# germannp/yalla

Hardware: AMD Instinct MI355X
Metric: cell-updates/sec at 1M cells (Grid_solver) (higher is better)
Workload: dtype f32

## Files before the change

include/solvers.cuh:

```cuda
#pragma once

#include <hip/hip_runtime.h>
#include <hip/hip_ext.h>

#include <assert.h>
#include <math.h>
#include <stdio.h>
#include <stdlib.h>
#include <string.h>

#include <functional>
#include <mutex>
#include <type_traits>
#include <utility>
#include <vector>

#include "cudebug.cuh"
#include "dtypes.cuh"
#include "fold256.cuh"
#include "yalla_hip.h"

#ifndef YALLA_NO_THRUST
#include <thrust/execution_policy.h>
#include <thrust/fill.h>
// ... 214 lines not shown

template<typename Pt>
__device__ __forceinline__ Pt store_rhs(
    Pt* __restrict__ d_dX, int i, bool has_gen, Pt F, float3 sum_v, float sum_friction)
{
    Pt dX;
    if (has_gen) {
        dX = d_dX[i];
        dX += F;
    } else {
        dX = F;
    }
    if (sum_friction > 0) {
        dX.x += sum_v.x / sum_friction;
        dX.y += sum_v.y / sum_friction;
        dX.z += sum_v.z / sum_friction;
    }
    d_dX[i] = dX;
    return dX;
}

template<typename Pt, Pairwise_interaction<Pt> pw_int, Pairwise_friction<Pt> pw_friction>
__device__ __forceinline__ void tile_pair(const Pt Xi, const Pt& Xj, const float3& vj, const int i, const int j, Pt& F,
    float3& sum_v, float& sum_friction)
{
    Pt r = Xi - Xj;
    float dist = dist3(r.x, r.y, r.z);
    F += pw_int(Xi, r, dist, i, j);
    float friction = pw_friction(Xi, r, dist, i, j);
    sum_friction += friction;
    if (friction != 0) {
        float3 v = vj;
        sum_v.x += friction * v.x;
        sum_v.y += friction * v.y;
        sum_v.z += friction * v.z;
    }
}

template<typename Pt, Pairwise_interaction<Pt> pw_int, Pairwise_friction<Pt> pw_friction>
__device__ __forceinline__ void tile_force_rows(const int n, const int block, const int id_base,
    const Pt* __restrict__ d_X, const float3* __restrict__ d_old_v, Pt* __restrict__ d_dX, const bool has_gen)
{
    __shared__ Pt sh_X[TILE_POINTS];
    __shared__ float3 sh_v[TILE_POINTS];

    const int local = block * TILE_BLOCK + threadIdx.x;
    const int i = id_base + local;
    Pt Xi = ya::zero<Pt>();
    if (local < n) Xi = d_X[local];
    Pt F = ya::zero<Pt>();
    float3 sum_v{0.f, 0.f, 0.f};
    float sum_friction = 0;
    for (int tile_start = 0; tile_start < n; tile_start += TILE_POINTS) {
        const int n_tile = min(TILE_POINTS, n - tile_start);
        __syncthreads();
        for (int k = threadIdx.x; k < n_tile; k += TILE_BLOCK) {
            sh_X[k] = d_X[tile_start + k];
            sh_v[k] = d_old_v[tile_start + k];
        }
        __syncthreads();
        if (local < n) {
#ifndef YA_TILE_UNROLL
#define YA_TILE_UNROLL 4
#endif
#pragma unroll YA_TILE_UNROLL
            for (int k = 0; k < n_tile; k++) {
                const int j = id_base + tile_start + k;
                tile_pair<Pt, pw_int, pw_friction>(Xi, sh_X[k], sh_v[k], i, j, F, sum_v, sum_friction);
            }
        }
    }
    if (local < n) store_rhs(d_dX, local, has_gen, F, sum_v, sum_friction);
}
template<typename Pt, Pairwise_interaction<Pt> pw_int, Pairwise_friction<Pt> pw_friction>
__global__ __launch_bounds__(TILE_BLOCK) void tile_force(const int n,
    const Pt* __restrict__ d_X, const float3* __restrict__ d_old_v, Pt* __restrict__ d_dX,
    const bool has_gen)
{
    tile_force_rows<Pt, pw_int, pw_friction>(n, blockIdx.x, 0, d_X, d_old_v, d_dX, has_gen);
}

template<typename Pt, Pairwise_interaction<Pt> pw_int, Pairwise_friction<Pt> pw_friction, int COOP_LANES>
__device__ __forceinline__ void tile_force_coop_rows(const int n, const int block, const int id_base,
    const Pt* __restrict__ d_X, const float3* __restrict__ d_old_v, Pt* __restrict__ d_dX, const bool has_gen)
{
    constexpr int COOP_CELLS = 256 / COOP_LANES;
    constexpr int NF = N_floats<Pt>::value;
    constexpr int NC = NF + 4;
    constexpr int TILE = (57344 / (COOP_CELLS * NC * 4)) / 64 * 64 > 512 ? 512 : (57344 / (COOP_CELLS * NC * 4)) / 64 * 64;
    static_assert(TILE >= 64, "point type too large for tile_force_coop");
    constexpr int THREADS = COOP_CELLS * COOP_LANES;
    constexpr int LOADS = (TILE + THREADS - 1) / THREADS;
    constexpr int SLOTS = (NC + COOP_LANES - 1) / COOP_LANES;
    __shared__ __attribute__((aligned(16))) float sh_part[COOP_CELLS][NC][TILE];
    __shared__ Pt sh_X[TILE];
    __shared__ float3 sh_v[TILE];
    __shared__ float sh_sum[COOP_CELLS][NC];

    const int cell = threadIdx.x / COOP_LANES, lane = threadIdx.x % COOP_LANES;
    const int local = block * COOP_CELLS + cell;
    const int i = id_base + local;
    const bool active = local < n;
    Pt Xi = ya::zero<Pt>();
    if (active) Xi = d_X[local];
    float acc[SLOTS];
#pragma unroll
    for (int a = 0; a < SLOTS; a++) acc[a] = 0.f;

    Pt x_next[LOADS];
    float3 v_next[LOADS];
#pragma unroll
    for (int k = 0; k < LOADS; k++) {
        const int j = threadIdx.x + k * THREADS;
        x_next[k] = ya::zero<Pt>();
        v_next[k] = float3{0.f, 0.f, 0.f};
        if (j < TILE && j < n) {
            x_next[k] = d_X[j];
            v_next[k] = d_old_v[j];
        }
    }
    for (int tile_start = 0; tile_start < n; tile_start += TILE) {
        const int n_tile = min(TILE, n - tile_start);
#pragma unroll
        for (int k = 0; k < LOADS; k++) {
            const int t = threadIdx.x + k * THREADS;
            if (t < TILE) {
                sh_X[t] = x_next[k];
                sh_v[t] = v_next[k];
                const int j_next = tile_start + TILE + t;
                if (j_next < n) {
                    x_next[k] = d_X[j_next];
                    v_next[k] = d_old_v[j_next];
                }
            }
        }
        __syncthreads();
        if (active) {
#pragma unroll 4
            for (int jj = lane; jj < n_tile; jj += COOP_LANES) {
                const int j = id_base + tile_start + jj;
                Pt r = Xi - sh_X[jj];
                float dist = dist3(r.x, r.y, r.z);
                const Pt f = pw_int(Xi, r, dist, i, j);
                const float friction = pw_friction(Xi, r, dist, i, j);
#pragma unroll
                for (int c = 0; c < NF; c++) sh_part[cell][c][jj] = field(f, c);
                sh_part[cell][NF][jj] = friction;
                const float3 v = sh_v[jj];
                sh_part[cell][NF + 1][jj] = friction != 0 ? friction * v.x : 0.f;
                sh_part[cell][NF + 2][jj] = friction != 0 ? friction * v.y : 0.f;
                sh_part[cell][NF + 3][jj] = friction != 0 ? friction * v.z : 0.f;
            }
        }
        __syncthreads();
#pragma unroll
        for (int a = 0; a < SLOTS; a++) {
            const int c = lane + COOP_LANES * a;
            if (c < NC && active) {
                float sum = acc[a];
                const float4* terms = reinterpret_cast<const float4*>(&sh_part[cell][c][0]);
                int jj = 0;
                for (; jj + 16 <= n_tile; jj += 16) {
                    float4 p[4];
#pragma unroll
                    for (int u = 0; u < 4; u++) p[u] = terms[jj / 4 + u];
#pragma unroll
                    for (int u = 0; u < 4; u++) {
                        sum += p[u].x;
                        sum += p[u].y;
                        sum += p[u].z;
                        sum += p[u].w;
                    }
                }
                for (; jj < n_tile; jj++) sum += sh_part[cell][c][jj];
                acc[a] = sum;
            }
        }
        __syncthreads();
    }
#pragma unroll
    for (int a = 0; a < SLOTS; a++) {
        const int c = lane + COOP_LANES * a;
        if (c < NC) sh_sum[cell][c] = acc[a];
    }
    __syncthreads();
    if (active && lane == 0) {
        Pt F;
#pragma unroll
        for (int c = 0; c < NF; c++) field(F, c) = sh_sum[cell][c];
        store_rhs(d_dX, local, has_gen, F,
            float3{sh_sum[cell][NF + 1], sh_sum[cell][NF + 2], sh_sum[cell][NF + 3]}, sh_sum[cell][NF]);
    }
}
template<typename Pt, Pairwise_interaction<Pt> pw_int, Pairwise_friction<Pt> pw_friction, int COOP_LANES>
__global__ __launch_bounds__(256) void tile_force_coop(const int n,
    const Pt* __restrict__ d_X, const float3* __restrict__ d_old_v, Pt* __restrict__ d_dX,
    const bool has_gen)
{
    tile_force_coop_rows<Pt, pw_int, pw_friction, COOP_LANES>(n, blockIdx.x, 0, d_X, d_old_v, d_dX, has_gen);
}

__device__ __forceinline__ int stencil_row_offset(int row, int gs)
{
    const int dy = row % 3, dz = row / 3;
    const int oy = dy == 0 ? 0 : (dy == 1 ? -gs : gs);
    const int oz = dz == 0 ? 0 : (dz == 1 ? -gs * gs : gs * gs);
    return oy + oz;
}


template<typename Pt>
__device__ __forceinline__ float4 staged_words(const Entry<Pt>* e)
{
    if constexpr (sizeof(Entry<Pt>) % 16 == 0)
        return *reinterpret_cast<const float4*>(e);
    else
        return float4{e->X.x, e->X.y, e->X.z, 0.f};
}
__device__ __forceinline__ void keep_wide(const float4& w) { asm volatile("" ::"v"(w.w)); }

template<typename Pt>
__device__ __forceinline__ float dist2_to(const Pt& a, const float4 b)
{
    const float dx = a.x - b.x;
    const float dy = a.y - b.y;
    const float dz = a.z - b.z;
    return fmaf(dz, dz, fmaf(dy, dy, dx * dx));
}

template<typename Pt>
__device__ __forceinline__ float dist2(const Pt& a, const Pt& b)
{
    const float dx = a.x - b.x;
    const float dy = a.y - b.y;
    const float dz = a.z - b.z;
    return fmaf(dz, dz, fmaf(dy, dy, dx * dx));
}

inline float cutoff_squared(float cube_size)
{
    float t = cube_size * cube_size;
    while (t > 0 && sqrtf(t) >= cube_size) t = nextafterf(t, 0.f);
    while (sqrtf(t) < cube_size) t = nextafterf(t, INFINITY);
    return t;
}

#ifndef YA_CALL_INLINED
#define YA_CALL_INLINED [[clang::always_inline]]
#endif

#define YA_ROW_BOUNDS(plane_)                                                          \
    _Pragma("unroll") for (int r = 0; r < 3; r++)                                      \
    {                                                                                  \
        const int off = stencil_row_offset(3 * (plane_) + r, gs);                      \
         \
         \
        next_lo[r] = offs[min(max(c_lo + off - 1, 0), n_cubes)];                       \
        next_hi[r] = offs[min(max(c_hi + off + 2, 0), n_cubes)];                       \
        next_begin[r] = offs[min(max(c + off - 1, 0), n_cubes)];                       \
        next_end[r] = offs[min(max(c + off + 2, 0), n_cubes)];                         \
    }

}
#ifdef YA_EXPERIMENTAL_FORCE_VARIANTS
#include "force_variants.cuh"
#endif
namespace ya {

template<typename Pt, Pairwise_friction<Pt> pw_friction>
__device__ __forceinline__ void pair_friction(const Pt& Xi, const Pt& r, const float dist, const int i,
    const int j, const float4& v, float3& sum_v, float& sum_friction)
{
    if constexpr (pw_friction == &friction_w_neighbour<Pt>) {
        const bool nb = (i != j) & (dist < 1.f);
        const float f = nb ? 1.f : 0.f;
        sum_friction += f;
        sum_v.x = fmaf(f, v.x, sum_v.x);
        sum_v.y = fmaf(f, v.y, sum_v.y);
        sum_v.z = fmaf(f, v.z, sum_v.z);
    } else {
        const float friction = pw_friction(Xi, r, dist, i, j);
        sum_friction += friction;
        if (friction != 0) {
            sum_v.x += friction * v.x;
            sum_v.y += friction * v.y;
            sum_v.z += friction * v.z;
        }
    }
}

#ifndef YA_BITS_PROBE_BEGIN
#define YA_BITS_PROBE_BEGIN
#define YA_BITS_PROBE_END(tile_)
#endif
namespace bits {
#ifndef YA_BITS_BLOCK
#define YA_BITS_BLOCK 64
#endif
#ifndef YA_MASK_WORDS
#define YA_MASK_WORDS 4
#endif
#ifndef YA_BITS_POPS
#define YA_BITS_POPS 2
#endif
#ifndef YA_BITS_POPS_WIDE
#define YA_BITS_POPS_WIDE 2
#endif
#ifndef YA_BITS_MIN_WAVES_WIDE
#define YA_BITS_MIN_WAVES_WIDE 1
#endif
template<typename Pt>
struct Min_waves {
    static constexpr int value = sizeof(Pt) <= 16 ? 1 : YA_BITS_MIN_WAVES_WIDE;
};
template<typename Pt>
struct Pops {
    static constexpr int value = sizeof(Pt) <= 16 ? YA_BITS_POPS : YA_BITS_POPS_WIDE;
};
constexpr int BLOCK = YA_BITS_BLOCK;
constexpr int WORDS = YA_MASK_WORDS;
constexpr int PASS_BITS = 32 * WORDS;
static_assert(BLOCK % 32 == 0, "phase 2 steps its word pointer by BLOCK / 32 elements per bit position");
using Lds_word = __attribute__((address_space(3))) unsigned;

template<typename Pt>
struct Stage {
#ifndef YA_BITS_STAGE_CELLS
#define YA_BITS_STAGE_CELLS (3 * YA_BITS_BLOCK + 160)
#endif
    static constexpr int value = sizeof(Entry<Pt>) <= 24 ? YA_BITS_STAGE_CELLS
                                 : (sizeof(Entry<Pt>) <= 32 ? 256 : YA_BITS_STAGE_CELLS / 2);
};

__device__ __forceinline__ void shift_in(unsigned& m, const float d2, const float cut2)
{
    asm("v_cmp_gt_f32 vcc, %2, %1\n\tv_addc_co_u32 %0, vcc, %0, %0, vcc"
        : "+v"(m)
        : "v"(d2), "s"(cut2)
        : "vcc");
}

__host__ __device__ constexpr bool offsets_fit_32_bits(const long long n)
{
    return n >= 0 && 16ll * n < (1ll << 32);
}

template<typename Pt, Pairwise_interaction<Pt> pw_int, Pairwise_friction<Pt> pw_friction, bool STAGE_V, bool GLOBAL_IDS,
    bool OFF32>
__device__ __forceinline__ void pass(const Entry<Pt>* __restrict__ sh_e, const float4* __restrict__ sh_v,
    Lds_word* const words,
    const int b0, const int e0, const int b1, const int e1, const int b2, const int e2,
    const int shift0, const int shift1, const int shift2, const float4* __restrict__ sorted_v,
    const Pt& Xi, const int i, const float cut2, Pt& F, float3& sum_v, float& sum_friction,
    const int* __restrict__ global_id, const int id_base = 0)
{
    constexpr int POPS = Pops<Pt>::value;
    unsigned m = 0;
    int p = 0;
    Lds_word* mp = words;
#define YA_BITS_GROUP(end_, masked_)                                                   \
    {                                                                                  \
        float4 w[4];                                                                   \
        float d2[4];                                                                   \
        _Pragma("unroll") for (int u = 0; u < 4; u++) w[u] = staged_words(&sh_e[t + u]); \
        _Pragma("unroll") for (int u = 0; u < 4; u++)                                  \
        {                                                                              \
            d2[u] = dist2_to(Xi, w[u]);                                                \
            keep_wide(w[u]);                                                           \
            if (masked_) d2[u] = t + u < (end_) ? d2[u] : INFINITY;                    \
        }                                                                              \
        _Pragma("unroll") for (int u = 0; u < 4; u++) shift_in(m, d2[u], cut2);        \
        p += 4;                                                                        \
        *mp = m;   \
        const bool full = (p & 31) == 0;                                               \
        mp += full ? BLOCK : 0;                                                        \
        m = full ? 0u : m;                                                             \
    }
#define YA_BITS_SEGMENT(begin_, end_)                                                  \
    {                                                                                  \
        int t = (begin_);                                                              \
        for (; t + 4 <= (end_); t += 4) YA_BITS_GROUP(end_, false)                     \
        if (t < (end_)) YA_BITS_GROUP(end_, true)                                      \
    }
    const int d0 = b0;
    YA_BITS_SEGMENT(b0, e0)
    const int p1 = p, d1 = b1 - p1;
    YA_BITS_SEGMENT(b1, e1)
    const int p2 = p, d2_ = b2 - p2;
    YA_BITS_SEGMENT(b2, e2)
#undef YA_BITS_SEGMENT
#undef YA_BITS_GROUP
    if (p & 31) *mp = m << (32 - (p & 31));

    constexpr unsigned ENTRY = sizeof(Entry<Pt>);
    constexpr bool ONE_OFFSET = ENTRY == sizeof(float4);
    const unsigned lds0 = ENTRY * (unsigned)d0, lds1 = ENTRY * (unsigned)d1, lds2 = ENTRY * (unsigned)d2_;
    const unsigned gat0 = 16u * (unsigned)(d0 + shift0), gat1 = 16u * (unsigned)(d1 + shift1),
                   gat2 = 16u * (unsigned)(d2_ + shift2);
    Lds_word* const rp_end = words + ((p + 31) >> 5) * BLOCK;
    unsigned cur = p > 0 ? words[0] : 0u;
    Lds_word* rp = words + BLOCK;
    unsigned nxt = *rp;
    int wbase = 0;
#define YA_BITS_LOAD(q_, other_, v_)                                                   \
    {                                                                                  \
        const bool in2 = (q_) >= p2, in1 = (q_) >= p1;                                 \
        if constexpr (OFF32 && ONE_OFFSET) {                                           \
            const unsigned at = ENTRY * (unsigned)(q_) + (in2 ? lds2 : (in1 ? lds1 : lds0)); \
            other_ = *(const Entry<Pt>*)((const char*)sh_e + at);                      \
            if (STAGE_V) v_ = *(const float4*)((const char*)sh_v + at);                \
        } else {                                                                       \
            const int t = (q_) + (in2 ? d2_ : (in1 ? d1 : d0));                        \
            other_ = sh_e[t];                                                          \
            if (STAGE_V) v_ = sh_v[t];                                                 \
            if (!STAGE_V && !OFF32) v_ = sorted_v[(unsigned)(t + (in2 ? shift2 : (in1 ? shift1 : shift0)))]; \
        }                                                                              \
        if constexpr (OFF32 && !STAGE_V) {                                             \
            const unsigned at = 16u * (unsigned)(q_) + (in2 ? gat2 : (in1 ? gat1 : gat0)); \
            v_ = *(const float4*)((const char*)sorted_v + (size_t)at);                 \
        }                                                                              \
    }
#define YA_BITS_PAIR(other_, v_)                                                       \
    {                                                                                  \
        Pt r = Xi - other_.X;                                                          \
        float dist = dist3(r.x, r.y, r.z);                                             \
        const int j = (GLOBAL_IDS ? global_id[other_.id] : other_.id) + id_base;       \
        YA_CALL_INLINED F += pw_int(Xi, r, dist, i, j);                                \
        pair_friction<Pt, pw_friction>(Xi, r, dist, i, j, v_, sum_v, sum_friction);    \
    }
#ifdef YA_BITS_MEASUREMENT_PROBES
#include "bits_probe.inc"
#endif
    while (cur != 0 || rp < rp_end) {
        const int step = cur == 0 ? 32 : 0;
        cur = cur == 0 ? nxt : cur;
        wbase += step;
        rp += step * (BLOCK / 32);
        nxt = *rp;
        if (cur != 0) {
            int pos[POPS];
            bool have[POPS];
            Entry<Pt> other[POPS];
            float4 v[POPS];
#pragma unroll
            for (int u = 0; u < POPS; u++) {
                have[u] = cur != 0;
                pos[u] = have[u] ? __builtin_clz(cur) : pos[u > 0 ? u - 1 : 0];
                cur = have[u] ? cur & (0x7fffffffu >> pos[u]) : cur;
                YA_BITS_LOAD(wbase + pos[u], other[u], v[u])
            }
            YA_BITS_PAIR(other[0], v[0])
#pragma unroll
            for (int u = 1; u < POPS; u++)
                if (have[u]) YA_BITS_PAIR(other[u], v[u])
        }
    }
#undef YA_BITS_LOAD
#undef YA_BITS_PAIR
}
}

template<typename Pt, Pairwise_interaction<Pt> pw_int, Pairwise_friction<Pt> pw_friction, bool STAGE_V, bool GLOBAL_IDS,
    bool OFF32>
__device__ __forceinline__ void grid_force_bits_tile(const int n, const int tile, const int id_base, const int half,
    const int slot, const Entry<Pt>* sorted, const float4* sorted_v,
    const int* cube_id, const int* offs, const int gs, const int n_cubes, const float cut2,
    Pt* d_dX, const bool has_gen, const int n_active, Pt* d_dX_sorted,
    const int* global_id, float* tail_exchange, int* tail_tickets, const bool by_plane);

template<typename Pt, Pairwise_interaction<Pt> pw_int, Pairwise_friction<Pt> pw_friction, bool STAGE_V = false,
    bool GLOBAL_IDS = false, bool OFF32 = true>
__global__ __launch_bounds__(bits::BLOCK, bits::Min_waves<Pt>::value) void grid_force_bits(const int n,
    const Entry<Pt>* __restrict__ sorted, const float4* __restrict__ sorted_v,
    const int* __restrict__ cube_id, const int* __restrict__ offs, const int gs,
    const int n_cubes, const float cut2, Pt* __restrict__ d_dX, const bool has_gen,
    const int n_active, Pt* __restrict__ d_dX_sorted, const int* __restrict__ global_id, const int n_tiles,
    const int tail, float* tail_exchange, int* tail_tickets, const bool by_plane,
    const int part = 0, const int part_cube_lo = 0, const int part_cube_hi = 0, const int own_cube_lo = 0,
    const int own_cube_hi = 0x7fffffff)
{
    constexpr int FB = bits::BLOCK;

    int tile, mine, t_first = 0, t_lo = 0, t_hi = 0;
    if (part == 0) {
        mine = n_tiles;
    } else {
        const int tiles = n_tiles;
        t_first = min(offs[min(max(own_cube_lo, 0), n_cubes)] / FB, tiles);
        const int t_end = max(min((offs[min(own_cube_hi, n_cubes)] + FB - 1) / FB, tiles), t_first);
        t_lo = max(min((offs[min(part_cube_lo, n_cubes)] + FB - 1) / FB, t_end), t_first);
        t_hi = max(min(offs[min(part_cube_hi, n_cubes)] / FB, t_end), t_lo);
        mine = part == 1 ? (t_lo - t_first) + (t_end - t_hi) : t_hi - t_lo;
    }
    const int whole = tail < 0 ? 0 : (tail > 0 && (part == 0 || mine >= 4 * tail) ? max(mine - tail, 0) & ~7 : mine);
    int half = -1, compact = blockIdx.x;
    if (compact >= whole) {
        const int b = compact - whole;
        half = (b >> 3) & 1;
        compact = whole + (b >> 4) * 8 + (b & 7);
    }
    if (compact >= mine) return;
    if (part == 0) {
        tile = xcd_contiguous_tile(compact, mine);
    } else {
        const int t = xcd_contiguous_tile<16>(compact, mine);
        if (part == 1)
            tile = t < t_lo - t_first ? t_first + t : t_hi + (t - (t_lo - t_first));
        else
            tile = t_lo + t;
    }
    grid_force_bits_tile<Pt, pw_int, pw_friction, STAGE_V, GLOBAL_IDS, OFF32>(n, tile, 0, half, compact - whole, sorted,
        sorted_v, cube_id, offs, gs, n_cubes, cut2, d_dX, has_gen, n_active, d_dX_sorted, global_id, tail_exchange,
        tail_tickets, by_plane);
}

template<typename Pt, Pairwise_interaction<Pt> pw_int, Pairwise_friction<Pt> pw_friction, bool STAGE_V, bool GLOBAL_IDS,
    bool OFF32>
__device__ __forceinline__ void grid_force_bits_tile(const int n, const int tile, const int id_base, const int half,
    const int slot, const Entry<Pt>* sorted, const float4* sorted_v,
    const int* cube_id, const int* offs, const int gs, const int n_cubes, const float cut2,
    Pt* d_dX, const bool has_gen, const int n_active, Pt* d_dX_sorted,
    const int* global_id, float* tail_exchange, int* tail_tickets, const bool by_plane)
{
    constexpr int FB = bits::BLOCK;
    constexpr int CAP = bits::Stage<Pt>::value;
    constexpr int NF = N_floats<Pt>::value;
    constexpr int NC = NF + 4;
    __shared__ __attribute__((aligned(16))) Entry<Pt> sh_e[CAP + 8];
    __shared__ unsigned sh_m[(bits::WORDS + 1) * FB];
    __shared__ float4 sh_v[STAGE_V ? CAP + 8 : 1];
    bits::Lds_word* const words = (bits::Lds_word*)sh_m + threadIdx.x;
    const int s0 = tile * FB;
    const int s = s0 + threadIdx.x;
    bool active = s < n;
    const int c_lo = cube_id[s0];
    const int c_hi = cube_id[min(s0 + FB, n) - 1];
    YA_BITS_PROBE_BEGIN

    Pt Xi = ya::zero<Pt>();
    int i = 0, c = c_lo;
    if (active) {
        const Entry<Pt> self = sorted[s];
        Xi = self.X;
        i = self.id;
        c = cube_id[s];
        active = i < n_active;
    }
    if (!__syncthreads_or(active)) return;
    const int gi = (GLOBAL_IDS && active ? global_id[i] : i) + id_base;
    Pt F = ya::zero<Pt>();
    float3 sum_v{0.f, 0.f, 0.f};
    float sum_friction = 0;

    constexpr bool OWN_IN_LDS = sizeof(Pt) > 16;
    __shared__ float sh_own[OWN_IN_LDS ? NC * FB : 1];
    float own[OWN_IN_LDS ? 1 : NC];
#pragma unroll
    for (int k = 0; k < (OWN_IN_LDS ? 1 : NC); k++) own[k] = 0.f;

    int next_lo[3], next_hi[3], next_begin[3], next_end[3];
    const int plane_first = half == 1 ? 1 : 0, plane_end = half == 0 ? 1 : 3;
#pragma unroll 1
    for (int plane = plane_first; plane < plane_end; plane++) {
        if (by_plane && half < 0 && plane == 1) {
            float save[NC];
#pragma unroll
            for (int k = 0; k < NF; k++) save[k] = field(F, k);
            save[NF] = sum_v.x, save[NF + 1] = sum_v.y, save[NF + 2] = sum_v.z, save[NF + 3] = sum_friction;
#pragma unroll
            for (int k = 0; k < NC; k++) {
                if (OWN_IN_LDS)
                    sh_own[k * FB + threadIdx.x] = save[k];
                else
                    own[OWN_IN_LDS ? 0 : k] = save[k];
            }
            F = ya::zero<Pt>(), sum_v = float3{0.f, 0.f, 0.f}, sum_friction = 0;
        }
        int wg_begin[3], v0[4], k_begin[3], k_end[3];
        v0[0] = 0;
        YA_ROW_BOUNDS(plane)
#pragma unroll
        for (int r = 0; r < 3; r++) {
            wg_begin[r] = next_lo[r];
            v0[r + 1] = v0[r] + next_hi[r] - wg_begin[r];
            k_begin[r] = next_begin[r];
            k_end[r] = active ? next_end[r] : k_begin[r];
        }
        const int total = v0[3];

        for (int chunk = 0; chunk < total; chunk += CAP) {
            const int chunk_n = min(CAP, total - chunk);
            __syncthreads();
            for (int t = threadIdx.x; t < chunk_n; t += FB) {
                const int v = chunk + t;
                const int shift = v >= v0[2] ? wg_begin[2] - v0[2]
                                             : (v >= v0[1] ? wg_begin[1] - v0[1] : wg_begin[0]);
                sh_e[t] = sorted[v + shift];
                if (STAGE_V) sh_v[t] = sorted_v[v + shift];
            }
            __syncthreads();
            int sb[3], se[3], shift[3];
#pragma unroll
            for (int r = 0; r < 3; r++) {
                sb[r] = max(k_begin[r] - wg_begin[r] + v0[r], chunk) - chunk;
                se[r] = min(k_end[r] - wg_begin[r] + v0[r], chunk + chunk_n) - chunk;
                shift[r] = wg_begin[r] - v0[r] + chunk;
            }
            const int bits_needed = (max(se[0] - sb[0], 0) + 3 & ~3) + (max(se[1] - sb[1], 0) + 3 & ~3) +
                                    (max(se[2] - sb[2], 0) + 3 & ~3);
            if (!__any(bits_needed > bits::PASS_BITS)) {
                bits::pass<Pt, pw_int, pw_friction, STAGE_V, GLOBAL_IDS, OFF32>(sh_e, sh_v, words, sb[0], se[0], sb[1], se[1], sb[2],
                    se[2], shift[0], shift[1], shift[2], sorted_v, Xi, gi, cut2, F, sum_v, sum_friction,
                    global_id, id_base);
            } else {
#pragma unroll 1
                for (int r = 0; r < 3; r++) {
                    const int rb = r == 0 ? sb[0] : (r == 1 ? sb[1] : sb[2]);
                    const int re = r == 0 ? se[0] : (r == 1 ? se[1] : se[2]);
                    const int rs = r == 0 ? shift[0] : (r == 1 ? shift[1] : shift[2]);
#pragma unroll 1
                    for (int b = rb; __any(b < re); b += bits::PASS_BITS)
                        bits::pass<Pt, pw_int, pw_friction, STAGE_V, GLOBAL_IDS, OFF32>(sh_e, sh_v, words, b, min(re, b + bits::PASS_BITS),
                            0, 0, 0, 0, rs, 0, 0, sorted_v, Xi, gi, cut2, F, sum_v, sum_friction, global_id, id_base);
                }
            }
        }
    }
    float sums[NC];
#pragma unroll
    for (int k = 0; k < NF; k++) sums[k] = field(F, k);
    sums[NF] = sum_v.x, sums[NF + 1] = sum_v.y, sums[NF + 2] = sum_v.z, sums[NF + 3] = sum_friction;
    if (half < 0) {
        if (by_plane) {
#pragma unroll
            for (int k = 0; k < NC; k++)
                sums[k] = (OWN_IN_LDS ? sh_own[k * FB + threadIdx.x] : own[OWN_IN_LDS ? 0 : k]) + sums[k];
        }
    } else {
        __shared__ int sh_second;
        float* const mine_out = tail_exchange + ((size_t)slot * 2 + half) * NC * FB + threadIdx.x;
#pragma unroll
        for (int k = 0; k < NC; k++)
            __hip_atomic_store(mine_out + k * FB, sums[k], __ATOMIC_RELAXED, __HIP_MEMORY_SCOPE_AGENT);
        asm volatile("s_waitcnt vmcnt(0)" ::: "memory");
        __syncthreads();
        if (threadIdx.x == 0)
            sh_second = __hip_atomic_fetch_add(&tail_tickets[slot], 1, __ATOMIC_RELAXED, __HIP_MEMORY_SCOPE_AGENT);
        __syncthreads();
        if (sh_second == 0) {
            YA_BITS_PROBE_END(tile)
            return;
        }
        if (threadIdx.x == 0) __hip_atomic_store(&tail_tickets[slot], 0, __ATOMIC_RELAXED, __HIP_MEMORY_SCOPE_AGENT);
        const float* const theirs = tail_exchange + ((size_t)slot * 2 + (1 - half)) * NC * FB + threadIdx.x;
#pragma unroll
        for (int k = 0; k < NC; k++)
            sums[k] = sums[k] + __hip_atomic_load(theirs + k * FB, __ATOMIC_RELAXED, __HIP_MEMORY_SCOPE_AGENT);
    }
    if (active) {
#pragma unroll
        for (int k = 0; k < NF; k++) field(F, k) = sums[k];
        const Pt dX = store_rhs(d_dX, i, has_gen, F, float3{sums[NF], sums[NF + 1], sums[NF + 2]}, sums[NF + 3]);
        if (d_dX_sorted) d_dX_sorted[s] = dX;
    }
    YA_BITS_PROBE_END(tile)
}


namespace coop {
constexpr int BLOCK = 256;
#ifndef YA_COOP_MAX_HITS
#define YA_COOP_MAX_HITS 96
#endif
constexpr int MAX_HITS = YA_COOP_MAX_HITS;
constexpr int STRETCH = 64;
template<typename Pt, int LANES>
struct Stage {
    static constexpr bool all_rows = sizeof(Entry<Pt>) <= 16 || (sizeof(Entry<Pt>) <= 32 && LANES == 16);
    static constexpr int value = (all_rows ? 9 : 5) * (BLOCK / LANES + 34);
};
inline int lanes_for(const int n, const bool by_plane = false)
{
    return n <= 15000 ? 16 : (n <= 40000 ? 8 : (n <= (by_plane ? 70000 : 120000) ? 4 : 1));
}
__device__ __forceinline__ void wave_sync()
{
    __builtin_amdgcn_fence(__ATOMIC_RELEASE, "wavefront");
    __builtin_amdgcn_wave_barrier();
    __builtin_amdgcn_fence(__ATOMIC_ACQUIRE, "wavefront");
}
}

template<typename Pt, Pairwise_interaction<Pt> pw_int, Pairwise_friction<Pt> pw_friction, int LANES>
__device__ __forceinline__ void grid_force_coop_cells(const int n, const int block, const int n_blocks,
    const int id_base, const Entry<Pt>* sorted, const float4* sorted_v,
    const int* cube_id, const int* offs, const int gs,
    const int n_cubes, const float cut2, Pt* d_dX, const bool has_gen,
    const int n_active, Pt* d_dX_sorted, const int* global_id, const bool by_plane)
{
    static_assert(LANES == 4 || LANES == 8 || LANES == 16, "lanes per cell");
    constexpr int CELLS = coop::BLOCK / LANES, MAX_HITS = coop::MAX_HITS;
    constexpr int CAP = coop::Stage<Pt, LANES>::value;
    static_assert(CAP < 4096, "a listed hit is row << 12 | LDS index");
    constexpr int NF = N_floats<Pt>::value;
    constexpr int NC = NF + 4;
    constexpr int SLOTS = (NC + LANES - 1) / LANES;
    constexpr bool STAGE_V = LANES >= 8;
    __shared__ __attribute__((aligned(16))) Entry<Pt> sh_e[CAP + 4];
    __shared__ float4 sh_v[STAGE_V ? CAP : 1];
    __shared__ unsigned short sh_hit[CELLS][MAX_HITS];
    __shared__ __attribute__((aligned(16))) float sh_term[CELLS][NC][LANES];
    __shared__ float sh_sum[CELLS][NC];
    __shared__ int sh_lo[9], sh_len[9], sh_shift[9], sh_kb[CELLS][9], sh_ke[CELLS][9];

    const int cell = threadIdx.x / LANES, lane = threadIdx.x % LANES;
    const int s0 = xcd_contiguous_tile(block, n_blocks) * CELLS;
    const int s = s0 + cell;
    bool active = s < n;

    Pt Xi = ya::zero<Pt>();
    int i = 0, c = 0;
    if (active) {
        const Entry<Pt> self = sorted[s];
        Xi = self.X;
        i = self.id;
        c = cube_id[s];
        active = i < n_active;
    }
    if (!__syncthreads_or(active)) return;
    const int gi = (global_id && active ? global_id[i] : i) + id_base;
    for (int r = lane; r < 9; r += LANES) {
        const int off = stencil_row_offset(r, gs);
        const int begin = offs[min(max(c + off - 1, 0), n_cubes)];
        sh_kb[cell][r] = begin;
        sh_ke[cell][r] = active ? offs[min(max(c + off + 2, 0), n_cubes)] : begin;
    }
    if (threadIdx.x < 9) {
        const int off = stencil_row_offset(threadIdx.x, gs);
        const int c_lo = cube_id[s0], c_hi = cube_id[min(s0 + CELLS, n) - 1];
        const int lo = offs[min(max(c_lo + off - 1, 0), n_cubes)];
        sh_lo[threadIdx.x] = lo;
        sh_len[threadIdx.x] = offs[min(max(c_hi + off + 2, 0), n_cubes)] - lo;
    }
    __syncthreads();
    int v0[10];
    v0[0] = 0;
#pragma unroll
    for (int r = 0; r < 9; r++) v0[r + 1] = v0[r] + sh_len[r];
    if (threadIdx.x < 9) {
        int mine = 0;
#pragma unroll
        for (int r = 0; r < 9; r++) mine = (int)threadIdx.x == r ? v0[r] : mine;
        sh_shift[threadIdx.x] = sh_lo[threadIdx.x] - mine;
    }
    __syncthreads();

    float acc[SLOTS];
    float acc_own[SLOTS];
#pragma unroll
    for (int a = 0; a < SLOTS; a++) acc[a] = 0.f, acc_own[a] = 0.f;
    bool own_done = !by_plane;
#define YA_COOP_OWN_DONE                                          \
    {                                                             \
        _Pragma("unroll") for (int a = 0; a < SLOTS; a++) acc_own[a] = acc[a], acc[a] = 0.f; \
        own_done = true;                                          \
    }

    const int rows_at_once = v0[9] <= CAP ? 9 : 3;
#pragma unroll 1
    for (int g0 = 0; g0 < 9; g0 += rows_at_once) {
        const int g_end = g0 + rows_at_once;
        if (g0 == 3 && !own_done) YA_COOP_OWN_DONE
        const int g_base = g0 == 0 ? 0 : (g0 == 3 ? v0[3] : v0[6]);
        const int g_total = (g_end == 9 ? v0[9] : (g_end == 3 ? v0[3] : v0[6])) - g_base;
#pragma unroll 1
        for (int chunk = 0; chunk < g_total; chunk += CAP) {
            const int chunk_n = min(CAP, g_total - chunk);
            const int base = g_base + chunk;
            __syncthreads();
            for (int t = threadIdx.x; t < chunk_n; t += coop::BLOCK) {
                const int v = base + t;
                int r = 0;
#pragma unroll
                for (int q = 1; q < 9; q++) r += v >= v0[q];
                const int slot = v + sh_shift[r];
                sh_e[t] = sorted[slot];
                if (STAGE_V) sh_v[t] = sorted_v[slot];
            }
            __syncthreads();

            int r = g0, sb, len, k0 = 0, sb_next, len_next;
#define YA_COOP_ROW(row_, sb_, len_)                                                   \
    {                                                                                  \
        const int rr = min(row_, 8);                                                   \
        const int shift = sh_shift[rr] + base;                                         \
        sb_ = max(sh_kb[cell][rr] - shift, 0);                                         \
        len_ = (row_) < g_end ? max(min(sh_ke[cell][rr] - shift, chunk_n) - sb_, 0) : 0; \
    }
            YA_COOP_ROW(g0, sb, len)
            YA_COOP_ROW(g0 + 1, sb_next, len_next)
            int listed = 0;
            while (true) {
                while (true) {
                    const int row_limit = own_done ? g_end : min(g_end, 3);
                    const int stretch = r < row_limit ? min(len - k0, coop::STRETCH) : 0;
                    const bool go = r < row_limit && listed + stretch <= MAX_HITS;
                    if (!__any(go)) break;
                    if (go) {
                        const int share = (stretch + LANES - 1) / LANES;
                        const int pb = sb + k0 + min(lane * share, stretch);
                        const int pe = sb + k0 + min(lane * share + share, stretch);
                        unsigned m = 0;
                        int bits = 0;
                        for (int t = pb; t < pe; t += 4) {
                            float4 w[4];
                            float d2[4];
#pragma unroll
                            for (int u = 0; u < 4; u++) w[u] = staged_words(&sh_e[t + u]);
#pragma unroll
                            for (int u = 0; u < 4; u++) {
                                d2[u] = dist2_to(Xi, w[u]);
                                keep_wide(w[u]);
                                d2[u] = t + u < pe ? d2[u] : INFINITY;
                            }
#pragma unroll
                            for (int u = 0; u < 4; u++) bits::shift_in(m, d2[u], cut2);
                            bits += 4;
                        }
                        m = bits > 0 ? m << (32 - bits) : 0u;
                        const int mine = __builtin_popcount(m);
                        int upto = mine;
#pragma unroll
                        for (int o = 1; o < LANES; o <<= 1) {
                            const int up = __shfl_up(upto, o, LANES);
                            upto += lane >= o ? up : 0;
                        }
                        int rank = listed + upto - mine;
                        listed += __shfl(upto, LANES - 1, LANES);
                        while (m != 0) {
                            const int pos = __builtin_clz(m);
                            m &= 0x7fffffffu >> pos;
                            sh_hit[cell][rank++] = (unsigned short)((r << 12) | (pb + pos));
                        }
                        k0 += stretch;
                        while (k0 >= len && r < g_end) {
                            r++;
                            k0 = 0;
                            sb = sb_next;
                            len = len_next;
                            YA_COOP_ROW(r + 1, sb_next, len_next)
                        }
                    }
                }
                if (!__any(listed > 0)) {
                    if (!__any(r < g_end)) break;
                    if (rows_at_once == 9 && !own_done && r >= 3) YA_COOP_OWN_DONE
                    continue;
                }
                coop::wave_sync();
                for (int h0 = 0; __any(h0 < listed); h0 += LANES) {
                    const int h = h0 + lane;
                    Pt f = ya::zero<Pt>();
                    float friction = 0;
                    float4 v{0.f, 0.f, 0.f, 0.f};
                    if (h < listed) {
                        const int e = sh_hit[cell][h];
                        const int t = e & 0xfff;
                        const Entry<Pt> other = sh_e[t];
                        if (STAGE_V)
                            v = sh_v[t];
                        else
                            v = sorted_v[(unsigned)(t + base + sh_shift[e >> 12])];
                        Pt rr = Xi - other.X;
                        float dist = dist3(rr.x, rr.y, rr.z);
                        const int j = (global_id ? global_id[other.id] : other.id) + id_base;
                        YA_CALL_INLINED f = pw_int(Xi, rr, dist, gi, j);
                        friction = pw_friction(Xi, rr, dist, gi, j);
                    }
#pragma unroll
                    for (int q = 0; q < NF; q++) sh_term[cell][q][lane] = field(f, q);
                    sh_term[cell][NF][lane] = friction;
                    sh_term[cell][NF + 1][lane] = friction != 0 ? friction * v.x : 0.f;
                    sh_term[cell][NF + 2][lane] = friction != 0 ? friction * v.y : 0.f;
                    sh_term[cell][NF + 3][lane] = friction != 0 ? friction * v.z : 0.f;
                    coop::wave_sync();
#pragma unroll
                    for (int a = 0; a < SLOTS; a++) {
                        const int q = lane + LANES * a;
                        if (q < NC) {
                            float sum = acc[a];
                            const float4* terms = reinterpret_cast<const float4*>(&sh_term[cell][q][0]);
#pragma unroll
                            for (int u = 0; u < LANES / 4; u++) {
                                const float4 p = terms[u];
                                sum += p.x;
                                sum += p.y;
                                sum += p.z;
                                sum += p.w;
                            }
                            acc[a] = sum;
                        }
                    }
                    coop::wave_sync();
                }
                listed = 0;
                if (rows_at_once == 9 && !own_done && r >= 3) YA_COOP_OWN_DONE
            }
#undef YA_COOP_ROW
        }
    }
#pragma unroll
    for (int a = 0; a < SLOTS; a++) {
        const int q = lane + LANES * a;
        if (q < NC) sh_sum[cell][q] = acc_own[a] + acc[a];
    }
#undef YA_COOP_OWN_DONE
    coop::wave_sync();
    if (active && lane == 0) {
        Pt F;
#pragma unroll
        for (int q = 0; q < NF; q++) field(F, q) = sh_sum[cell][q];
        const Pt dX = store_rhs(d_dX, i, has_gen, F,
            float3{sh_sum[cell][NF + 1], sh_sum[cell][NF + 2], sh_sum[cell][NF + 3]}, sh_sum[cell][NF]);
        if (d_dX_sorted) d_dX_sorted[s] = dX;
    }
// ... 1494 lines not shown
```

Measured before the change: 866.4 million.

## Streamline bitmask build phase and stage neighbor cells directly into LDS

Rewrites the first phase of the bitmask pass to walk each segment with byte offsets and compute the mask word address from a running counter OR'd with the thread's LDS column. This drops the per-group bounds masking and the full-word bookkeeping, and the tail is masked once at the end. The staging loop now uses global_load_lds to copy sorted entries (and velocities) straight into shared memory without going through registers, followed by an explicit vmcnt wait. A ONE_SEGMENT specialization is used for the fallback per-row passes. The address trick requires the mask buffer to be aligned, and the direct path only applies to 16-byte entries with 64-thread blocks.

```diff
diff --git a/include/solvers.cuh b/include/solvers.cuh
--- a/include/solvers.cuh
+++ b/include/solvers.cuh
@@ -540,6 +540,12 @@
 #endif
 #ifndef YA_BITS_POPS
 #define YA_BITS_POPS 2
+#endif
+#ifndef YA_BITS_LEAN_PHASE1
+#define YA_BITS_LEAN_PHASE1 1
+#endif
+#ifndef YA_BITS_STAGE_DIRECT
+#define YA_BITS_STAGE_DIRECT 1
 #endif
 #ifndef YA_BITS_POPS_WIDE
 #define YA_BITS_POPS_WIDE 2
@@ -584,7 +590,7 @@
 }
 
 template<typename Pt, Pairwise_interaction<Pt> pw_int, Pairwise_friction<Pt> pw_friction, bool STAGE_V, bool GLOBAL_IDS,
-    bool OFF32>
+    bool OFF32, bool ONE_SEGMENT = false>
 __device__ __forceinline__ void pass(const Entry<Pt>* __restrict__ sh_e, const float4* __restrict__ sh_v,
     Lds_word* const words,
     const int b0, const int e0, const int b1, const int e1, const int b2, const int e2,
@@ -592,8 +598,50 @@
     const Pt& Xi, const int i, const float cut2, Pt& F, float3& sum_v, float& sum_friction,
     const int* __restrict__ global_id, const int id_base = 0)
 {
-    constexpr int POPS = Pops<Pt>::value;
+    constexpr int POPS = ONE_SEGMENT ? 1 : Pops<Pt>::value;
     unsigned m = 0;
+#if YA_BITS_LEAN_PHASE1
+    constexpr unsigned GROUP = 4 * sizeof(Entry<Pt>);
+    constexpr unsigned STRIDE = 4 * BLOCK;
+    static_assert((STRIDE & (STRIDE - 1)) == 0 && STRIDE % 32 == 0, "the word's offset is a masked bit count");
+    const unsigned column = (unsigned)(__UINTPTR_TYPE__)words;
+    const int p1 = max(e0 - b0, 0) + 3 & ~3, p2 = ONE_SEGMENT ? p1 : p1 + (max(e1 - b1, 0) + 3 & ~3);
+    const int p = ONE_SEGMENT ? p1 : p2 + (max(e2 - b2, 0) + 3 & ~3);
+#define YA_BITS_SEGMENT(begin_, end_, p_begin_)                                        \
+    if ((begin_) < (end_)) {                                                           \
+        unsigned at = (unsigned)sizeof(Entry<Pt>) * (unsigned)(begin_);                \
+        const unsigned at_end = (unsigned)sizeof(Entry<Pt>) * (unsigned)(end_);        \
+        unsigned count = (STRIDE / 32) * (unsigned)(p_begin_);                         \
+        unsigned word;                                                                 \
+        do {                                                                           \
+            float4 w[4];                                                               \
+            float d2[4];                                                               \
+            _Pragma("unroll") for (int u = 0; u < 4; u++)                              \
+                w[u] = staged_words((const Entry<Pt>*)((const char*)sh_e + at) + u);   \
+            _Pragma("unroll") for (int u = 0; u < 4; u++)                              \
+            {                                                                          \
+                d2[u] = dist2_to(Xi, w[u]);                                            \
+                keep_wide(w[u]);                                                       \
+            }                                                                          \
+            _Pragma("unroll") for (int u = 0; u < 4; u++) shift_in(m, d2[u], cut2);    \
+            word = (count & ~(STRIDE - 1)) | column;                                   \
+            *(Lds_word*)(__UINTPTR_TYPE__)word = m;                                    \
+            count += STRIDE / 8;                                                       \
+            at += GROUP;                                                               \
+        } while (at < at_end);                                                         \
+        m &= ~0u << (at - at_end) / (unsigned)sizeof(Entry<Pt>);  \
+        *(Lds_word*)(__UINTPTR_TYPE__)word = m;                                        \
+    }
+    const int d0 = b0;
+    YA_BITS_SEGMENT(b0, e0, 0)
+    const int d1 = b1 - p1, d2_ = b2 - p2;
+    if constexpr (!ONE_SEGMENT) {
+        YA_BITS_SEGMENT(b1, e1, p1)
+        YA_BITS_SEGMENT(b2, e2, p2)
+    }
+#undef YA_BITS_SEGMENT
+    if (p & 31) words[(p >> 5) * BLOCK] = m << (32 - (p & 31));
+#else
     int p = 0;
     Lds_word* mp = words;
 #define YA_BITS_GROUP(end_, masked_)                                                   \
@@ -629,6 +677,7 @@
 #undef YA_BITS_SEGMENT
 #undef YA_BITS_GROUP
     if (p & 31) *mp = m << (32 - (p & 31));
+#endif
 
     constexpr unsigned ENTRY = sizeof(Entry<Pt>);
     constexpr bool ONE_OFFSET = ENTRY == sizeof(float4);
@@ -642,7 +691,7 @@
     int wbase = 0;
 #define YA_BITS_LOAD(q_, other_, v_)                                                   \
     {                                                                                  \
-        const bool in2 = (q_) >= p2, in1 = (q_) >= p1;                                 \
+        const bool in2 = !ONE_SEGMENT && (q_) >= p2, in1 = !ONE_SEGMENT && (q_) >= p1; \
         if constexpr (OFF32 && ONE_OFFSET) {                                           \
             const unsigned at = ENTRY * (unsigned)(q_) + (in2 ? lds2 : (in1 ? lds1 : lds0)); \
             other_ = *(const Entry<Pt>*)((const char*)sh_e + at);                      \
@@ -765,7 +814,7 @@
     constexpr int NF = N_floats<Pt>::value;
     constexpr int NC = NF + 4;
     __shared__ __attribute__((aligned(16))) Entry<Pt> sh_e[CAP + 8];
-    __shared__ unsigned sh_m[(bits::WORDS + 1) * FB];
+    __shared__ __attribute__((aligned(4 * FB))) unsigned sh_m[(bits::WORDS + 1) * FB];
     __shared__ float4 sh_v[STAGE_V ? CAP + 8 : 1];
     bits::Lds_word* const words = (bits::Lds_word*)sh_m + threadIdx.x;
     const int s0 = tile * FB;
@@ -829,12 +878,30 @@
         for (int chunk = 0; chunk < total; chunk += CAP) {
             const int chunk_n = min(CAP, total - chunk);
             __syncthreads();
-            for (int t = threadIdx.x; t < chunk_n; t += FB) {
-                const int v = chunk + t;
-                const int shift = v >= v0[2] ? wg_begin[2] - v0[2]
-                                             : (v >= v0[1] ? wg_begin[1] - v0[1] : wg_begin[0]);
-                sh_e[t] = sorted[v + shift];
-                if (STAGE_V) sh_v[t] = sorted_v[v + shift];
+            if constexpr (YA_BITS_STAGE_DIRECT && sizeof(Entry<Pt>) == 16 && FB == 64) {
+                using Global = const __attribute__((address_space(1))) void*;
+                using Lds = __attribute__((address_space(3))) void*;
+#pragma unroll
+                for (int k = 0; k < (CAP + FB - 1) / FB; k++) {
+                    const int lane = threadIdx.x, first = chunk + k * FB;
+                    if (lane < chunk_n - k * FB) {
+                        const int slot = lane + (lane >= v0[2] - first ? wg_begin[2] - v0[2] + first
+                                                 : (lane >= v0[1] - first ? wg_begin[1] - v0[1] + first
+                                                                          : wg_begin[0] + first));
+                        __builtin_amdgcn_global_load_lds((Global)&sorted[slot], (Lds)&sh_e[k * FB], 16, 0, 0);
+                        if (STAGE_V)
+                            __builtin_amdgcn_global_load_lds((Global)&sorted_v[slot], (Lds)&sh_v[k * FB], 16, 0, 0);
+                    }
+                }
+                asm volatile("s_waitcnt vmcnt(0)" ::: "memory");
+            } else {
+                for (int t = threadIdx.x; t < chunk_n; t += FB) {
+                    const int v = chunk + t;
+                    const int shift = v >= v0[2] ? wg_begin[2] - v0[2]
+                                                 : (v >= v0[1] ? wg_begin[1] - v0[1] : wg_begin[0]);
+                    sh_e[t] = sorted[v + shift];
+                    if (STAGE_V) sh_v[t] = sorted_v[v + shift];
+                }
             }
             __syncthreads();
             int sb[3], se[3], shift[3];
@@ -858,7 +925,7 @@
                     const int rs = r == 0 ? shift[0] : (r == 1 ? shift[1] : shift[2]);
 #pragma unroll 1
                     for (int b = rb; __any(b < re); b += bits::PASS_BITS)
-                        bits::pass<Pt, pw_int, pw_friction, STAGE_V, GLOBAL_IDS, OFF32>(sh_e, sh_v, words, b, min(re, b + bits::PASS_BITS),
+                        bits::pass<Pt, pw_int, pw_friction, STAGE_V, GLOBAL_IDS, OFF32, YA_BITS_LEAN_PHASE1>(sh_e, sh_v, words, b, min(re, b + bits::PASS_BITS),
                             0, 0, 0, 0, rs, 0, 0, sorted_v, Xi, gi, cut2, F, sum_v, sum_friction, global_id, id_base);
                 }
             }
```

Result: no change. 871.9 million, median of 6 (+0.6%).
